# verdurin/pbdagcon

Hardware: AMD Instinct MI355X
Metric: consensus bases/sec (whole node) (higher is better)
Workload: dtype u8

## Files before the change

pbdagcon_amd/csrc/k_build.hip.h:

```cpp
#pragma once
#include <hip/hip_runtime.h>
#include "dagcon_dev.h"

#define DG_WAVE 64
#ifndef DG_LPW
#define DG_LPW 8u
#endif

__device__ __forceinline__ bool dg_failed(const DgParams &p) {
    return __hip_atomic_load(&p.st->err_flags, __ATOMIC_RELAXED, __HIP_MEMORY_SCOPE_AGENT) != 0;
}
__device__ __forceinline__ void dg_fail(const DgParams &p, uint32_t bit) {
    atomicOr(&p.st->err_flags, bit);
}
__device__ __forceinline__ void dg_fail_target(const DgParams &p, uint32_t t, uint32_t bit) {
    atomicOr(&p.tfail[t], bit);
}
__device__ __forceinline__ bool dg_tskip(const DgParams &p, uint32_t t) {
    return !p.tactive[t] || __hip_atomic_load(&p.tfail[t], __ATOMIC_RELAXED, __HIP_MEMORY_SCOPE_AGENT) != 0;
}
__device__ __forceinline__ bool dg_askip(const DgParams &p, uint32_t a) {
    return !(p.flags & DG_F_A1_ONLY) && __hip_atomic_load(&p.tfail[p.aln_tgt[a]], __ATOMIC_RELAXED, __HIP_MEMORY_SCOPE_AGENT) != 0;
}
__device__ __forceinline__ void dg_fail_aln(const DgParams &p, uint32_t a, uint32_t bit) {
    if (p.flags & DG_F_A1_ONLY) dg_fail(p, bit);
    else dg_fail_target(p, p.aln_tgt[a], bit);
    p.st->bad_aln = a;
}

#define DG_COL(qb, tb) ((uint16_t)((uint16_t)(qb) | ((uint16_t)(tb) << 8)))
#define DG_Q(c) ((uint8_t)((c) & 0xff))
#define DG_T(c) ((uint8_t)((c) >> 8))
#define DG_NW 64u
#define DG_NW_BIG 512u
#define DG_REDO 0xFFFFFFFFu

template <typename CT>
__device__ __forceinline__ void dg_store_run(const DgParams &p, CT *cell, const uint32_t run) {
    if constexpr (sizeof(CT) == 1) {
        if (run > 255u) { dg_fail(p, DG_E_RUN_WIDE); return; }
    }
    *cell = (CT)run;
}

template <typename CT>
__device__ inline void dg_finish_alignment(const DgParams &p, uint32_t a, uint16_t *buf, uint32_t m) {
    const uint32_t trim = p.trim;
    uint32_t lbases = 0, rbases = 0, lo = 0, hi = m;
    uint32_t start = p.aln_start[a];
    while (lbases < trim && lo < m) {
        if (DG_T(buf[lo++]) != DG_GAP) lbases++;
    }
    while (rbases < trim && hi > lo) {
        if (DG_T(buf[--hi]) != DG_GAP) rbases++;
    }
    start += lbases;
    const bool graph = !(p.flags & DG_F_A1_ONLY);
    uint32_t t_idx = 0, r = 0;
    CT *Cm = nullptr;
    if (graph) {
        t_idx = p.aln_tgt[a];
        if (p.tactive[t_idx]) {
            const uint64_t ab = p.aln_begin[t_idx];
            r = (uint32_t)(a - ab);
            Cm = static_cast<CT *>(p.matC) + p.matc_base[t_idx] + (uint64_t)r * p.matc_stride[t_idx];
        }
    }
    const uint32_t tlen = graph ? p.tlen[t_idx] : 0xFFFFFFFFu;
    uint32_t n_ins = 0, n_del = 0, adv = 0, run = 0;
    bool conf = start >= 1;
    uint32_t i = lo;
#define DG_FIN_COL(c, ci_)                                                                \
    do {                                                                                  \
        const uint8_t qb_ = DG_Q(c), tb_ = DG_T(c);                                       \
        if (qb_ == tb_ || qb_ == DG_GAP) {                                                \
            if (Cm && conf && ((start + adv) & ((1u << p.emit_shift) - 1u)) == 0 && start + adv <= tlen + 1) \
                ck[(start + adv) >> p.emit_shift] = ci_ - run;                            \
            if (run) { if (Cm && conf && start + adv <= tlen + 1) dg_store_run(p, Cm + (start + adv), run); run = 0; } \
            adv++; n_del += (qb_ != tb_);                                                 \
            if ((uint64_t)start - 1 + adv > (uint64_t)tlen) conf = false;                 \
        } else if (tb_ == DG_GAP) { n_ins++; run++; }                                     \
    } while (0)
    uint32_t *ck = p.ckpt + p.ck_base[a];
    while (i < hi && (i & 7u)) { const uint16_t c = buf[i]; DG_FIN_COL(c, i); i++; }
    while (i + 8 <= hi) {
        const uint4 v = *reinterpret_cast<const uint4 *>(buf + i);
        const uint32_t w4[4] = {v.x, v.y, v.z, v.w};
#pragma unroll
        for (int k = 0; k < 4; k++) {
            const uint16_t c0 = (uint16_t)(w4[k] & 0xffffu), c1 = (uint16_t)(w4[k] >> 16);
            DG_FIN_COL(c0, i + 2 * k);
            DG_FIN_COL(c1, i + 2 * k + 1);
        }
        i += 8;
    }
    while (i < hi) { const uint16_t c = buf[i]; DG_FIN_COL(c, i); i++; }
    if (run && Cm && conf && ((start + adv) & ((1u << p.emit_shift) - 1u)) == 0 && start + adv <= tlen + 1)
        ck[(start + adv) >> p.emit_shift] = hi - run;
    if (run && Cm && conf && start + adv <= tlen + 1) dg_store_run(p, Cm + (start + adv), run);
#undef DG_FIN_COL
    p.n_lo[a] = lo; p.n_hi[a] = hi; p.n_start[a] = start;
    p.n_ins[a] = n_ins; p.n_del[a] = n_del;
    atomicAdd(&p.st->n_columns, (unsigned long long)(hi - lo));
    if (graph && hi > lo && !conf) dg_fail_aln(p, a, DG_E_NONCONF);
}

#ifndef DG_NCH
#define DG_NCH 512u
#endif
#define DG_CH_NONE 0xFFFFFFFFu

__device__ __forceinline__ bool dg_match_col(uint8_t qb, uint8_t tb) { return qb == tb && qb != DG_GAP && qb != '.'; }

__device__ inline uint32_t dg_chunk_start(const uint8_t *q, const uint8_t *t, uint32_t len, uint32_t c) {
    if (c == 0) return 0;
    const uint64_t w0 = (uint64_t)c * DG_NCH;
    if (w0 >= len) return DG_CH_NONE;
    const uint32_t hi = (uint64_t)len < w0 + DG_NCH ? len : (uint32_t)(w0 + DG_NCH);
    for (uint32_t k = (uint32_t)w0; k < hi; k++) {
        const uint8_t b = q[k];
        if (dg_match_col(b, t[k]) && b != q[k - 1] && dg_match_col(q[k - 1], t[k - 1]) && dg_match_col(q[k - 2], t[k - 2]))
            return k;
    }
    return DG_CH_NONE;
}

struct DgChunkRun { uint32_t w, tb; bool dirty, overflow, badchar; };

template <uint32_t NW>
__device__ inline DgChunkRun dg_norm_run(const uint8_t *q, const uint8_t *t, const uint32_t len, const uint32_t k0,
                                         const uint32_t k1, uint16_t *win, uint16_t *out) {
#define DG_W(x) win[(x) & (NW - 1u)]
    DgChunkRun r;
    r.w = 0; r.tb = 0; r.dirty = false; r.overflow = false; r.badchar = false;
    if (k0 >= k1) return r;
    uint32_t badw = 0;
    uint32_t ip = k0, e = 0, i = 0, w = 0, tb = 0, jt = 0, jq = 0;
    uint32_t e_end = 0xFFFFFFFFu;
    uint32_t o0 = 0, o1 = 0, o2 = 0, o3 = 0;
    uint32_t in_done = 0, dirty = 0, overflow = 0;
    for (;;) {
        asm volatile("" : "+v"(in_done), "+v"(dirty));
        if (!in_done && (e - i) + 32u > NW) { overflow = 1; break; }
        if (!in_done) {
            uint32_t take = len - ip;
            if (take > 16u) take = 16u;
            if (ip < k1 && take > k1 - ip) take = k1 - ip;
#define DG_EXPAND(QB, TB)                                                      \
            do {                                                               \
                uint8_t qb_ = (QB), tb_ = (TB);                                \
                if (qb_ == '.') qb_ = DG_GAP;                                  \
                if (tb_ == '.') tb_ = DG_GAP;                                  \
                 \
                                   \
                const bool mm_ = qb_ != tb_ && qb_ != DG_GAP && tb_ != DG_GAP; \
                DG_W(e) = mm_ ? DG_COL(DG_GAP, tb_) : DG_COL(qb_, tb_);        \
                DG_W(e + 1u) = DG_COL(qb_, DG_GAP);                            \
                e += mm_ ? 2u : 1u;                                            \
            } while (0)
            if (take == 16u && (((uintptr_t)(q + ip)) & 15u) == 0) {
                const uint4 qv = *reinterpret_cast<const uint4 *>(q + ip);
                const uint4 tv = *reinterpret_cast<const uint4 *>(t + ip);
                const uint32_t qw[4] = {qv.x, qv.y, qv.z, qv.w}, tw[4] = {tv.x, tv.y, tv.z, tv.w};
#pragma unroll
                for (int k = 0; k < 4; k++) {
                    badw |= ((qw[k] - 0x21212121u) & ~qw[k]) | ((qw[k] + 0x01010101u) | qw[k]);
                    badw |= ((tw[k] - 0x21212121u) & ~tw[k]) | ((tw[k] + 0x01010101u) | tw[k]);
                }
#pragma unroll
                for (int k = 0; k < 16; k++)
                    DG_EXPAND((uint8_t)(qw[k >> 2] >> (8 * (k & 3))), (uint8_t)(tw[k >> 2] >> (8 * (k & 3))));
            } else {
                const uint32_t to_align = (uint32_t)((16u - (((uintptr_t)(q + ip)) & 15u)) & 15u);
                if (to_align && take > to_align) take = to_align;
                for (uint32_t k = 0; k < take; k++) {
                    const uint8_t qb0 = q[ip + k], tb0 = t[ip + k];
                    if (qb0 < 33 || qb0 > 126 || tb0 < 33 || tb0 > 126) badw = 0x80u;
                    DG_EXPAND(qb0, tb0);
                }
            }
#undef DG_EXPAND
            ip += take;
            if (ip == k1) e_end = e;
            if (ip == len) in_done = 1;
        }
        while (i < e && i < e_end) {
            if (i + 1 == e && !in_done) break;
            const uint16_t c = DG_W(i);
            uint8_t qi = DG_Q(c), ti = DG_T(c);
            uint32_t more = 0;
            if (i + 1 < e) {
                if (ti == DG_GAP) {
                    if (jt <= i) jt = i + 1;
                    while (jt < e && DG_T(DG_W(jt)) == DG_GAP) jt++;
                    if (jt < e) {
                        const uint16_t cj = DG_W(jt);
                        if (DG_T(cj) == qi) { ti = qi; DG_W(jt) = DG_COL(DG_Q(cj), DG_GAP); dirty |= (uint32_t)(jt >= e_end); }
                    } else if (!in_done) more = 2;
                }
                if (!more && qi == DG_GAP) {
                    if (jq <= i) jq = i + 1;
                    while (jq < e && DG_Q(DG_W(jq)) == DG_GAP) jq++;
                    if (jq < e) {
                        const uint16_t cj = DG_W(jq);
                        if (DG_Q(cj) == ti) { qi = ti; DG_W(jq) = DG_COL(DG_GAP, DG_T(cj)); dirty |= (uint32_t)(jq >= e_end); }
                    } else if (!in_done) more = 2;
                }
            }
            if (more) { DG_W(i) = DG_COL(qi, ti); break; }
            if (qi != DG_GAP || ti != DG_GAP) {
                o0 = (o0 >> 16) | (o1 << 16); o1 = (o1 >> 16) | (o2 << 16); o2 = (o2 >> 16) | (o3 << 16);
                o3 = (o3 >> 16) | ((uint32_t)DG_COL(qi, ti) << 16);
                w++;
                tb += (ti != DG_GAP);
                if ((w & 7u) == 0) *reinterpret_cast<uint4 *>(out + w - 8) = make_uint4(o0, o1, o2, o3);
            }
            i++;
        }
        if (i == e_end) break;
    }
#undef DG_W
    for (uint32_t k = w & 7u, x = w - (w & 7u); k > 0; k--, x++) {
        const uint32_t sh = 8u - k;
        const uint32_t word = sh >> 1;
        const uint32_t v = word == 0 ? o0 : word == 1 ? o1 : word == 2 ? o2 : o3;
        out[x] = (uint16_t)((sh & 1u) ? v >> 16 : v & 0xffffu);
    }
    r.w = w; r.tb = tb; r.dirty = dirty != 0; r.overflow = overflow != 0; r.badchar = (badw & 0x80808080u) != 0;
    return r;
}

template <uint32_t NW, uint32_t LANES, bool RETRY>
__global__ __launch_bounds__(LANES) void k_norm_chunk(DgParams p) {
    __shared__ uint16_t s_win[LANES * (NW + 2u)];
    const uint32_t g = threadIdx.x * gridDim.x + blockIdx.x;
    if (g >= p.n_chunks) return;
    if (dg_failed(p)) return;
    if (RETRY && p.ch_flag[g] != 2u) return;
    const uint32_t a = p.ch_aln[g];
    if (dg_askip(p, a)) { if (!RETRY) p.ch_flag[g] = 0; return; }
    const uint32_t c = g - p.ch_base[a], nwin = p.ch_base[a + 1] - p.ch_base[a];
    const uint64_t off = p.aln_off[a];
    const uint32_t len = p.aln_len[a];
    const uint8_t *q = p.q + off, *t = p.t + off;
    uint32_t flag = 0;
    DgChunkRun r;
    r.w = 0; r.tb = 0; r.dirty = false; r.overflow = false; r.badchar = false;
    uint32_t k0 = DG_CH_NONE, cn = c + 1;
    uint64_t src = 0;
    if (p.flags & DG_F_RAW) {
        if (c == 0) { k0 = 0; cn = nwin; flag = 1; }
    } else {
        k0 = dg_chunk_start(q, t, len, c);
        if (k0 != DG_CH_NONE) {
            uint16_t *win = s_win + threadIdx.x * (NW + 2u);
            src = (2ull * (off + k0) + 8ull * g + 7ull) & ~7ull;
            for (;;) {
                uint32_t k1 = len;
                for (; cn < nwin; cn++) {
                    const uint32_t s = dg_chunk_start(q, t, len, cn);
                    if (s != DG_CH_NONE) { k1 = s; break; }
                }
                r = dg_norm_run<NW>(q, t, len, k0, k1, win, p.norm_tmp + src);
                if (r.badchar) dg_fail_aln(p, a, DG_E_BADCHAR);
                if (r.overflow) { flag = RETRY ? 1u : 2u; break; }
                if (!r.dirty) break;
                cn++;
                uint32_t k2 = len;
                for (uint32_t x = cn; x < nwin; x++) {
                    const uint32_t s = dg_chunk_start(q, t, len, x);
                    if (s != DG_CH_NONE) { k2 = s; break; }
                }
                const unsigned long long need = (2ull * (k2 - k0) + 15ull) & ~7ull;
                const unsigned long long o = atomicAdd(&p.st->ovf_top, need);
                if (p.tmp_main + o + need > p.tmp_cap) { flag = 1; break; }
                src = p.tmp_main + o;
            }
        }
    }
    p.ch_k0[g] = k0; p.ch_next[g] = cn; p.ch_w[g] = r.w; p.ch_tb[g] = r.tb;
    p.ch_flag[g] = flag; p.ch_src[g] = src;
}

__global__ __launch_bounds__(64) void k_norm_scan(DgParams p) {
    const uint32_t a = blockIdx.x * 64 + threadIdx.x;
    if (a >= p.A) return;
    if (dg_failed(p)) return;
    if (dg_askip(p, a)) return;
    const uint32_t g0 = p.ch_base[a], g1 = p.ch_base[a + 1];
    bool redo = false;
    uint32_t m = 0, tbt = 0;
    for (uint32_t g = g0; g < g1;) {
        if (p.ch_k0[g] == DG_CH_NONE) { p.ch_out[g] = DG_CH_NONE; g++; continue; }
        redo |= p.ch_flag[g] != 0;
        p.ch_out[g] = m; p.ch_adv[g] = tbt;
        m += p.ch_w[g]; tbt += p.ch_tb[g];
        uint32_t nx = g0 + p.ch_next[g];
        if (nx > g1) nx = g1;
        for (uint32_t x = g + 1; x < nx; x++) p.ch_out[x] = DG_CH_NONE;
        g = nx;
    }
    if (redo) { p.n_hi[a] = DG_REDO; return; }
    const uint32_t trim = p.trim;
    uint32_t lbases = 0, rbases = 0, lo = 0, hi = m;
    for (uint32_t g = g0; g < g1 && lbases < trim && lo < m; g++) {
        if (p.ch_out[g] == DG_CH_NONE) continue;
        const uint32_t w = p.ch_w[g], tb = p.ch_tb[g];
        if (lbases + tb < trim) { lo += w; lbases += tb; continue; }
        const uint16_t *src = p.norm_tmp + p.ch_src[g];
        for (uint32_t x = 0; x < w && lbases < trim; x++) {
            if (DG_T(src[x]) != DG_GAP) lbases++;
            lo++;
        }
    }
    for (uint32_t g = g1; g > g0 && rbases < trim && hi > lo;) {
        g--;
        const uint32_t o = p.ch_out[g];
        if (o == DG_CH_NONE) continue;
        const uint32_t tb = p.ch_tb[g];
        if (o >= lo && rbases + tb < trim) { hi = o; rbases += tb; continue; }
        const uint16_t *src = p.norm_tmp + p.ch_src[g];
        while (rbases < trim && hi > lo && hi > o) {
            if (DG_T(src[--hi - o]) != DG_GAP) rbases++;
        }
    }
    p.n_lo[a] = lo; p.n_hi[a] = hi; p.n_start[a] = p.aln_start[a] + lbases; p.n_lb[a] = lbases;
    p.n_ins[a] = 0; p.n_del[a] = 0;
    atomicAdd(&p.st->n_columns, (unsigned long long)(hi - lo));
}

__device__ __forceinline__ uint4 dg_funnel_cols(const uint4 A, const uint4 B, const uint32_t h) {
    const bool w1 = (h >> 1) & 1u, w2 = (h >> 2) & 1u, half = h & 1u;
    const uint32_t u0 = w1 ? A.y : A.x, u1 = w1 ? A.z : A.y, u2 = w1 ? A.w : A.z, u3 = w1 ? B.x : A.w,
                   u4 = w1 ? B.y : B.x, u5 = w1 ? B.z : B.y, u6 = w1 ? B.w : B.z;
    const uint32_t t0 = w2 ? u2 : u0, t1 = w2 ? u3 : u1, t2 = w2 ? u4 : u2, t3 = w2 ? u5 : u3, t4 = w2 ? u6 : u4;
    uint4 r;
    r.x = half ? __builtin_amdgcn_alignbit(t1, t0, 16) : t0;
    r.y = half ? __builtin_amdgcn_alignbit(t2, t1, 16) : t1;
    r.z = half ? __builtin_amdgcn_alignbit(t3, t2, 16) : t2;
    r.w = half ? __builtin_amdgcn_alignbit(t4, t3, 16) : t3;
    return r;
}

__device__ __forceinline__ uint32_t dg_wave_excl(const uint32_t v, const int lane) {
    int incl = (int)v;
    incl += __builtin_amdgcn_update_dpp(0, incl, 0x111, 0xf, 0xf, false);
    incl += __builtin_amdgcn_update_dpp(0, incl, 0x112, 0xf, 0xf, false);
    incl += __builtin_amdgcn_update_dpp(0, incl, 0x114, 0xf, 0xf, false);
    incl += __builtin_amdgcn_update_dpp(0, incl, 0x118, 0xf, 0xf, false);
    incl += __builtin_amdgcn_update_dpp(0, incl, 0x142, 0xa, 0xf, false);
    incl += __builtin_amdgcn_update_dpp(0, incl, 0x143, 0xc, 0xf, false);
    (void)lane;
    return (uint32_t)incl - v;
}

template <typename CT>
__global__ __launch_bounds__(256) void k_norm_finish2(DgParams p) {
    const uint32_t g = blockIdx.x * 4u + (threadIdx.x >> 6);
    if (g >= p.n_chunks) return;
    if (dg_failed(p)) return;
    const int lane = threadIdx.x & 63;
    const uint32_t a = p.ch_aln[g];
    if (dg_askip(p, a)) return;
    const uint32_t o = p.ch_out[g];
    if (o == DG_CH_NONE) return;
    const uint32_t hi = p.n_hi[a];
    if (hi == DG_REDO) return;
    const uint32_t lo = p.n_lo[a], start = p.n_start[a], lb = p.n_lb[a];
    const uint32_t w = p.ch_w[g], adv0 = p.ch_adv[g];
    const uint16_t *src = p.norm_tmp + p.ch_src[g];
    const uint4 *src4 = reinterpret_cast<const uint4 *>(src);
    uint16_t *dst = p.norm + p.norm_off[a] + o;
    const bool graph = !(p.flags & DG_F_A1_ONLY);
    uint32_t t_idx = 0;
    CT *Cm = nullptr;
    if (graph) {
        t_idx = p.aln_tgt[a];
        if (p.tactive[t_idx]) Cm = static_cast<CT *>(p.matC) + p.matc_base[t_idx] + (uint64_t)(a - p.aln_begin[t_idx]) * p.matc_stride[t_idx];
    }
    const uint32_t tlen = graph ? p.tlen[t_idx] : 0xFFFFFFFFu;
    uint32_t *ck = p.ckpt + p.ck_base[a];
    const uint32_t ck_mask = (1u << p.emit_shift) - 1u;
    const uint32_t adv_init = adv0 > lb ? adv0 - lb : 0u;
    const uint32_t f0 = lo > o ? lo - o : 0u;
    const uint32_t f1 = hi > o ? (hi - o < w ? hi - o : w) : 0u;
    const bool any = f1 > f0;
    const uint32_t fspan = any ? f1 - f0 : 0u;
#define DG_FIN_CONF(A) (start >= 1u && ((A) == 0u || (uint64_t)start - 1u + (A) <= (uint64_t)tlen))
    const uint32_t h0 = (8u - (o & 7u)) & 7u;
    const uint32_t h = h0 < w ? h0 : w;
    const uint32_t nb = (w - h) / 8u, nvec = (w + 7u) / 8u;
    if ((uint32_t)lane < h) dst[lane] = src[lane];
    { const uint32_t x = h + 8u * nb + (uint32_t)lane; if (lane < 8 && x < w) dst[x] = src[x]; }
    uint4 *dst4 = reinterpret_cast<uint4 *>(dst + h);
    uint32_t adv_tile = adv_init, run_tile = 0, n_ins = 0, n_del = 0;
    for (uint32_t v0 = 0; v0 < nvec; v0 += 64u) {
        const uint32_t vl = v0 + (uint32_t)lane;
        const uint4 pc = vl < nvec ? src4[vl] : make_uint4(0, 0, 0, 0);
        const uint4 pn = vl + 1 < nvec ? src4[vl + 1] : make_uint4(0, 0, 0, 0);
        if (vl < nb) dst4[vl] = dg_funnel_cols(pc, pn, h);
        if (!any || 8u * v0 >= f1) continue;
        uint32_t advm = 0, insm = 0, delm = 0;
#pragma unroll
        for (uint32_t k = 0; k < 8u; k++) {
            const uint32_t wd = ((k >> 1) & 3u) == 0 ? pc.x : ((k >> 1) & 3u) == 1 ? pc.y : ((k >> 1) & 3u) == 2 ? pc.z : pc.w;
            const uint16_t c = (uint16_t)((k & 1u) ? wd >> 16 : wd & 0xffffu);
            const bool inw = 8u * vl + k < 8u * nvec && 8u * vl + k - f0 < fspan;
            const uint8_t qb = DG_Q(c), tb = DG_T(c);
            const bool adv = inw && (qb == tb || qb == DG_GAP);
            advm |= adv ? 1u << k : 0u;
            delm |= (adv && qb != tb) ? 1u << k : 0u;
            insm |= (inw && !adv && tb == DG_GAP) ? 1u << k : 0u;
        }
        const uint32_t nadv = (uint32_t)__popc(advm), nI = (uint32_t)__popc(insm);
        n_ins += nI; n_del += (uint32_t)__popc(delm);
        const uint32_t adv_lane = adv_tile + dg_wave_excl(nadv, lane);
        uint32_t sf = advm ? 1u : 0u;
        uint32_t sv = advm ? (uint32_t)__popc(insm & ~((2u << (31 - __clz((int)advm))) - 1u)) : nI;
#pragma unroll
        for (int d = 1; d < 64; d <<= 1) {
            const uint32_t pf = (uint32_t)__shfl_up((int)sf, d), pv = (uint32_t)__shfl_up((int)sv, d);
            if (lane >= d) { sv = sf ? sv : pv + sv; sf |= pf; }
        }
        uint32_t ef = (uint32_t)__shfl_up((int)sf, 1), ev = (uint32_t)__shfl_up((int)sv, 1);
        if (lane == 0) { ef = 0; ev = 0; }
        uint32_t run = ef ? ev : ev + run_tile;
        const uint32_t lf = (uint32_t)__builtin_amdgcn_readlane((int)sf, 63), lv = (uint32_t)__builtin_amdgcn_readlane((int)sv, 63);
        run_tile = lf ? lv : lv + run_tile;
        adv_tile += (uint32_t)__builtin_amdgcn_readlane((int)(adv_lane - adv_tile + nadv), 63);
        uint32_t adv = adv_lane;
        if (Cm && (advm | insm)) {
#pragma unroll
            for (uint32_t k = 0; k < 8u; k++) {
                if ((advm >> k) & 1u) {
                    const bool conf = DG_FIN_CONF(adv);
                    const uint32_t x = 8u * vl + k;
                    if (conf && ((start + adv) & ck_mask) == 0 && start + adv <= tlen + 1 && !(x == 0 && o > lo))
                        ck[(start + adv) >> p.emit_shift] = o + x - run;
                    if (run && conf && start + adv <= tlen + 1) dg_store_run(p, Cm + (start + adv), run);
                    run = 0;
                    adv++;
                } else if ((insm >> k) & 1u) run++;
            }
        }
    }
    {
        const uint32_t adv = adv_tile, run = run_tile;
        const bool conf = DG_FIN_CONF(adv);
        if (lane == 0) {
            if (any && Cm && conf && ((start + adv) & ck_mask) == 0 && start + adv <= tlen + 1 && (o + f1 < hi || run))
                ck[(start + adv) >> p.emit_shift] = o + f1 - run;
            if (run && Cm && conf && start + adv <= tlen + 1) dg_store_run(p, Cm + (start + adv), run);
            if (graph && any && !conf) dg_fail_aln(p, a, DG_E_NONCONF);
        }
    }
    {
        const uint32_t ti = dg_wave_excl(n_ins, lane) + n_ins, td = dg_wave_excl(n_del, lane) + n_del;
        if (lane == 63) { if (ti) atomicAdd(&p.n_ins[a], ti); if (td) atomicAdd(&p.n_del[a], td); }
    }
#undef DG_FIN_CONF
}

template <typename CT>
__global__ __launch_bounds__(64) void k_normalize_slow(DgParams p) {
    const uint32_t a = blockIdx.x * 64 + threadIdx.x;
    if (a >= p.A) return;
    if (dg_failed(p)) return;
    if (dg_askip(p, a)) return;
    if (p.n_hi[a] != DG_REDO) return;
    const uint64_t off = p.aln_off[a];
    const uint32_t len = p.aln_len[a];
    const uint8_t *q = p.q + off, *t = p.t + off;
    uint16_t *buf = p.norm + p.norm_off[a];
    const bool raw = (p.flags & DG_F_RAW) != 0;
    uint32_t n = 0;
    for (uint32_t i = 0; i < len; i++) {
        uint8_t qb = q[i], tb = t[i];
        if (qb < 33 || qb > 126 || tb < 33 || tb > 126) dg_fail_aln(p, a, DG_E_BADCHAR);
        if (!raw) {
            if (qb == '.') qb = DG_GAP;
            if (tb == '.') tb = DG_GAP;
            if (qb != tb && qb != DG_GAP && tb != DG_GAP) {
                buf[n++] = DG_COL(DG_GAP, tb);
                buf[n++] = DG_COL(qb, DG_GAP);
                continue;
            }
        }
        buf[n++] = DG_COL(qb, tb);
    }
    uint32_t m = n;
    if (!raw) {
        uint32_t w = 0, jt = 0, jq = 0;
        for (uint32_t i = 0; i < n; i++) {
            uint16_t c = buf[i];
            uint8_t qi = DG_Q(c), ti = DG_T(c);
            if (i + 1 < n) {
                if (ti == DG_GAP) {
                    if (jt <= i) jt = i + 1;
                    while (jt < n && DG_T(buf[jt]) == DG_GAP) jt++;
                    if (jt < n) {
                        uint16_t cj = buf[jt];
                        if (DG_T(cj) == qi) { ti = qi; buf[jt] = DG_COL(DG_Q(cj), DG_GAP); }
                    }
                }
                if (qi == DG_GAP) {
                    if (jq <= i) jq = i + 1;
                    while (jq < n && DG_Q(buf[jq]) == DG_GAP) jq++;
                    if (jq < n) {
                        uint16_t cj = buf[jq];
                        if (DG_Q(cj) == ti) { qi = ti; buf[jq] = DG_COL(DG_GAP, DG_T(cj)); }
                    }
                }
            }
            if (qi != DG_GAP || ti != DG_GAP) buf[w++] = DG_COL(qi, ti);
        }
        m = w;
    }
    dg_finish_alignment<CT>(p, a, buf, m);
}

__device__ __forceinline__ uint32_t dg_pool_words(uint32_t tlen, uint32_t n_ins, uint32_t n_del,
                                                  uint32_t k, uint32_t growth_pct, uint32_t *fixed_words) {
    const uint64_t capb = dg_capb(k);
    const uint64_t fixed = 3ull * n_ins + (uint64_t)(tlen + 2) * 3ull * capb;
    const uint64_t spill = 3ull * ((uint64_t)n_ins + n_del + 2ull * k) + 64ull;
    const uint64_t growth = (fixed * growth_pct) / 100ull + spill + 256ull;
    *fixed_words = (uint32_t)fixed;
    const uint64_t tot = fixed + growth;
    return tot > 0xFFFFFFF0ull ? 0xFFFFFFF0u : (uint32_t)tot;
}

__global__ __launch_bounds__(1024) void k_carve(DgParams p) {
    __shared__ unsigned long long s_scan[1024];
    __shared__ unsigned long long s_carry_nodes, s_carry_pool;
    if (dg_failed(p)) return;
    const uint32_t tid = threadIdx.x;
    if (tid == 0) { s_carry_nodes = 0; s_carry_pool = 0; }
    __syncthreads();
    for (uint32_t t0 = 0; t0 < p.T; t0 += 1024) {
        const uint32_t t = t0 + tid;
        unsigned long long nodes = 0, poolw = 0;
        uint32_t fixed_words = 0, ins = 0;
        if (t < p.T && !dg_tskip(p, t)) {
            uint32_t del = 0;
            const uint64_t b = p.aln_begin[t], e = p.aln_begin[t + 1];
            for (uint64_t a = b; a < e; a++) { ins += p.n_ins[a]; del += p.n_del[a]; }
            nodes = (unsigned long long)p.tlen[t] + 2ull + ins;
            poolw = dg_pool_words(p.tlen[t], ins, del, (uint32_t)(e - b), p.growth_pct, &fixed_words);
            if (nodes > DG_MAX_NODES || poolw > 0x3FFFFFFFull) {
                dg_fail_target(p, t, DG_E_TOO_BIG);
                nodes = 0; poolw = 0; fixed_words = 0;
            }
        }
        s_scan[tid] = nodes;
        __syncthreads();
        for (uint32_t o = 1; o < 1024; o <<= 1) {
            unsigned long long v = tid >= o ? s_scan[tid - o] : 0;
            __syncthreads();
            s_scan[tid] += v;
            __syncthreads();
        }
        unsigned long long node_excl = s_scan[tid] - nodes + s_carry_nodes;
        unsigned long long node_tot = s_scan[1023];
        __syncthreads();
        s_scan[tid] = poolw;
        __syncthreads();
// ... 752 lines not shown
```

Before: 350.3 million.

## Add bitmask gap-skipping normalization run for the 64-slot window path

Adds a new normalization routine for the default 64-entry window. It keeps per-column target-gap and query-gap bitmasks and uses ctz to jump straight to gap columns and their partners, instead of scanning every column with per-byte branches. Input expansion is rewritten with SWAR byte-compare masks, and output is emitted in 8-column blocks with a fast path for gap-free blocks. The kernel also gains a launch-bounds occupancy hint for the non-retry variant. The bit logic is intricate and could diverge from the original scan on edge cases. The tighter occupancy hint may force register spills.

```diff
diff --git a/pbdagcon_amd/csrc/k_build.hip.h b/pbdagcon_amd/csrc/k_build.hip.h
--- a/pbdagcon_amd/csrc/k_build.hip.h
+++ b/pbdagcon_amd/csrc/k_build.hip.h
@@ -1,6 +1,7 @@
 #pragma once
 #include <hip/hip_runtime.h>
 #include "dagcon_dev.h"
+#include "k_norm_run.hip.h"
 
 #define DG_WAVE 64
 #ifndef DG_LPW
@@ -28,9 +29,6 @@
     p.st->bad_aln = a;
 }
 
-#define DG_COL(qb, tb) ((uint16_t)((uint16_t)(qb) | ((uint16_t)(tb) << 8)))
-#define DG_Q(c) ((uint8_t)((c) & 0xff))
-#define DG_T(c) ((uint8_t)((c) >> 8))
 #define DG_NW 64u
 #define DG_NW_BIG 512u
 #define DG_REDO 0xFFFFFFFFu
@@ -105,133 +103,8 @@
     if (graph && hi > lo && !conf) dg_fail_aln(p, a, DG_E_NONCONF);
 }
 
-#ifndef DG_NCH
-#define DG_NCH 512u
-#endif
-#define DG_CH_NONE 0xFFFFFFFFu
-
-__device__ __forceinline__ bool dg_match_col(uint8_t qb, uint8_t tb) { return qb == tb && qb != DG_GAP && qb != '.'; }
-
-__device__ inline uint32_t dg_chunk_start(const uint8_t *q, const uint8_t *t, uint32_t len, uint32_t c) {
-    if (c == 0) return 0;
-    const uint64_t w0 = (uint64_t)c * DG_NCH;
-    if (w0 >= len) return DG_CH_NONE;
-    const uint32_t hi = (uint64_t)len < w0 + DG_NCH ? len : (uint32_t)(w0 + DG_NCH);
-    for (uint32_t k = (uint32_t)w0; k < hi; k++) {
-        const uint8_t b = q[k];
-        if (dg_match_col(b, t[k]) && b != q[k - 1] && dg_match_col(q[k - 1], t[k - 1]) && dg_match_col(q[k - 2], t[k - 2]))
-            return k;
-    }
-    return DG_CH_NONE;
-}
-
-struct DgChunkRun { uint32_t w, tb; bool dirty, overflow, badchar; };
-
-template <uint32_t NW>
-__device__ inline DgChunkRun dg_norm_run(const uint8_t *q, const uint8_t *t, const uint32_t len, const uint32_t k0,
-                                         const uint32_t k1, uint16_t *win, uint16_t *out) {
-#define DG_W(x) win[(x) & (NW - 1u)]
-    DgChunkRun r;
-    r.w = 0; r.tb = 0; r.dirty = false; r.overflow = false; r.badchar = false;
-    if (k0 >= k1) return r;
-    uint32_t badw = 0;
-    uint32_t ip = k0, e = 0, i = 0, w = 0, tb = 0, jt = 0, jq = 0;
-    uint32_t e_end = 0xFFFFFFFFu;
-    uint32_t o0 = 0, o1 = 0, o2 = 0, o3 = 0;
-    uint32_t in_done = 0, dirty = 0, overflow = 0;
-    for (;;) {
-        asm volatile("" : "+v"(in_done), "+v"(dirty));
-        if (!in_done && (e - i) + 32u > NW) { overflow = 1; break; }
-        if (!in_done) {
-            uint32_t take = len - ip;
-            if (take > 16u) take = 16u;
-            if (ip < k1 && take > k1 - ip) take = k1 - ip;
-#define DG_EXPAND(QB, TB)                                                      \
-            do {                                                               \
-                uint8_t qb_ = (QB), tb_ = (TB);                                \
-                if (qb_ == '.') qb_ = DG_GAP;                                  \
-                if (tb_ == '.') tb_ = DG_GAP;                                  \
-                 \
-                                   \
-                const bool mm_ = qb_ != tb_ && qb_ != DG_GAP && tb_ != DG_GAP; \
-                DG_W(e) = mm_ ? DG_COL(DG_GAP, tb_) : DG_COL(qb_, tb_);        \
-                DG_W(e + 1u) = DG_COL(qb_, DG_GAP);                            \
-                e += mm_ ? 2u : 1u;                                            \
-            } while (0)
-            if (take == 16u && (((uintptr_t)(q + ip)) & 15u) == 0) {
-                const uint4 qv = *reinterpret_cast<const uint4 *>(q + ip);
-                const uint4 tv = *reinterpret_cast<const uint4 *>(t + ip);
-                const uint32_t qw[4] = {qv.x, qv.y, qv.z, qv.w}, tw[4] = {tv.x, tv.y, tv.z, tv.w};
-#pragma unroll
-                for (int k = 0; k < 4; k++) {
-                    badw |= ((qw[k] - 0x21212121u) & ~qw[k]) | ((qw[k] + 0x01010101u) | qw[k]);
-                    badw |= ((tw[k] - 0x21212121u) & ~tw[k]) | ((tw[k] + 0x01010101u) | tw[k]);
-                }
-#pragma unroll
-                for (int k = 0; k < 16; k++)
-                    DG_EXPAND((uint8_t)(qw[k >> 2] >> (8 * (k & 3))), (uint8_t)(tw[k >> 2] >> (8 * (k & 3))));
-            } else {
-                const uint32_t to_align = (uint32_t)((16u - (((uintptr_t)(q + ip)) & 15u)) & 15u);
-                if (to_align && take > to_align) take = to_align;
-                for (uint32_t k = 0; k < take; k++) {
-                    const uint8_t qb0 = q[ip + k], tb0 = t[ip + k];
-                    if (qb0 < 33 || qb0 > 126 || tb0 < 33 || tb0 > 126) badw = 0x80u;
-                    DG_EXPAND(qb0, tb0);
-                }
-            }
-#undef DG_EXPAND
-            ip += take;
-            if (ip == k1) e_end = e;
-            if (ip == len) in_done = 1;
-        }
-        while (i < e && i < e_end) {
-            if (i + 1 == e && !in_done) break;
-            const uint16_t c = DG_W(i);
-            uint8_t qi = DG_Q(c), ti = DG_T(c);
-            uint32_t more = 0;
-            if (i + 1 < e) {
-                if (ti == DG_GAP) {
-                    if (jt <= i) jt = i + 1;
-                    while (jt < e && DG_T(DG_W(jt)) == DG_GAP) jt++;
-                    if (jt < e) {
-                        const uint16_t cj = DG_W(jt);
-                        if (DG_T(cj) == qi) { ti = qi; DG_W(jt) = DG_COL(DG_Q(cj), DG_GAP); dirty |= (uint32_t)(jt >= e_end); }
-                    } else if (!in_done) more = 2;
-                }
-                if (!more && qi == DG_GAP) {
-                    if (jq <= i) jq = i + 1;
-                    while (jq < e && DG_Q(DG_W(jq)) == DG_GAP) jq++;
-                    if (jq < e) {
-                        const uint16_t cj = DG_W(jq);
-                        if (DG_Q(cj) == ti) { qi = ti; DG_W(jq) = DG_COL(DG_GAP, DG_T(cj)); dirty |= (uint32_t)(jq >= e_end); }
-                    } else if (!in_done) more = 2;
-                }
-            }
-            if (more) { DG_W(i) = DG_COL(qi, ti); break; }
-            if (qi != DG_GAP || ti != DG_GAP) {
-                o0 = (o0 >> 16) | (o1 << 16); o1 = (o1 >> 16) | (o2 << 16); o2 = (o2 >> 16) | (o3 << 16);
-                o3 = (o3 >> 16) | ((uint32_t)DG_COL(qi, ti) << 16);
-                w++;
-                tb += (ti != DG_GAP);
-                if ((w & 7u) == 0) *reinterpret_cast<uint4 *>(out + w - 8) = make_uint4(o0, o1, o2, o3);
-            }
-            i++;
-        }
-        if (i == e_end) break;
-    }
-#undef DG_W
-    for (uint32_t k = w & 7u, x = w - (w & 7u); k > 0; k--, x++) {
-        const uint32_t sh = 8u - k;
-        const uint32_t word = sh >> 1;
-        const uint32_t v = word == 0 ? o0 : word == 1 ? o1 : word == 2 ? o2 : o3;
-        out[x] = (uint16_t)((sh & 1u) ? v >> 16 : v & 0xffffu);
-    }
-    r.w = w; r.tb = tb; r.dirty = dirty != 0; r.overflow = overflow != 0; r.badchar = (badw & 0x80808080u) != 0;
-    return r;
-}
-
 template <uint32_t NW, uint32_t LANES, bool RETRY>
-__global__ __launch_bounds__(LANES) void k_norm_chunk(DgParams p) {
+__global__ __launch_bounds__(LANES, RETRY ? 1 : 5) void k_norm_chunk(DgParams p) {
     __shared__ uint16_t s_win[LANES * (NW + 2u)];
     const uint32_t g = threadIdx.x * gridDim.x + blockIdx.x;
     if (g >= p.n_chunks) return;
@@ -261,7 +134,8 @@
                     const uint32_t s = dg_chunk_start(q, t, len, cn);
                     if (s != DG_CH_NONE) { k1 = s; break; }
                 }
-                r = dg_norm_run<NW>(q, t, len, k0, k1, win, p.norm_tmp + src);
+                if constexpr (NW == DG_NW) r = dg_norm_run_gc(q, t, len, k0, k1, win, p.norm_tmp + src);
+                else r = dg_norm_run<NW>(q, t, len, k0, k1, win, p.norm_tmp + src);
                 if (r.badchar) dg_fail_aln(p, a, DG_E_BADCHAR);
                 if (r.overflow) { flag = RETRY ? 1u : 2u; break; }
                 if (!r.dirty) break;
diff --git a/pbdagcon_amd/csrc/k_norm_run.hip.h b/pbdagcon_amd/csrc/k_norm_run.hip.h
--- /dev/null
+++ b/pbdagcon_amd/csrc/k_norm_run.hip.h
@@ -0,0 +1,309 @@
+#pragma once
+#include <stddef.h>
+#include <stdint.h>
+
+#if defined(__HIPCC__)
+#include <hip/hip_runtime.h>
+#define DG_HD __host__ __device__
+#define DG_HD_INLINE __host__ __device__ __forceinline__
+typedef uint4 dg_u4;
+#define DG_MAKE_U4(a, b, c, d) make_uint4((a), (b), (c), (d))
+#else
+#define DG_HD
+#define DG_HD_INLINE inline __attribute__((always_inline))
+struct __attribute__((may_alias, aligned(16))) dg_u4 { uint32_t x, y, z, w; };
+static inline dg_u4 DG_MAKE_U4(uint32_t a, uint32_t b, uint32_t c, uint32_t d) { dg_u4 v; v.x = a; v.y = b; v.z = c; v.w = d; return v; }
+#endif
+#ifndef DG_GAP
+#define DG_GAP '-'
+#endif
+
+#define DG_COL(qb, tb) ((uint16_t)((uint16_t)(qb) | ((uint16_t)(tb) << 8)))
+#define DG_Q(c) ((uint8_t)((c) & 0xff))
+#define DG_T(c) ((uint8_t)((c) >> 8))
+
+#ifndef DG_NCH
+#define DG_NCH 512u
+#endif
+#define DG_CH_NONE 0xFFFFFFFFu
+
+DG_HD_INLINE bool dg_match_col(uint8_t qb, uint8_t tb) { return qb == tb && qb != DG_GAP && qb != '.'; }
+
+DG_HD inline uint32_t dg_chunk_start(const uint8_t *q, const uint8_t *t, uint32_t len, uint32_t c) {
+    if (c == 0) return 0;
+    const uint64_t w0 = (uint64_t)c * DG_NCH;
+    if (w0 >= len) return DG_CH_NONE;
+    const uint32_t hi = (uint64_t)len < w0 + DG_NCH ? len : (uint32_t)(w0 + DG_NCH);
+    for (uint32_t k = (uint32_t)w0; k < hi; k++) {
+        const uint8_t b = q[k];
+        if (dg_match_col(b, t[k]) && b != q[k - 1] && dg_match_col(q[k - 1], t[k - 1]) && dg_match_col(q[k - 2], t[k - 2]))
+            return k;
+    }
+    return DG_CH_NONE;
+}
+
+struct DgChunkRun { uint32_t w, tb; bool dirty, overflow, badchar; };
+
+template <uint32_t NW>
+DG_HD inline DgChunkRun dg_norm_run(const uint8_t *q, const uint8_t *t, const uint32_t len, const uint32_t k0,
+                                    const uint32_t k1, uint16_t *win, uint16_t *out) {
+#define DG_W(x) win[(x) & (NW - 1u)]
+    DgChunkRun r;
+    r.w = 0; r.tb = 0; r.dirty = false; r.overflow = false; r.badchar = false;
+    if (k0 >= k1) return r;
+    uint32_t badw = 0;
+    uint32_t ip = k0, e = 0, i = 0, w = 0, tb = 0, jt = 0, jq = 0;
+    uint32_t e_end = 0xFFFFFFFFu;
+    uint32_t o0 = 0, o1 = 0, o2 = 0, o3 = 0;
+    uint32_t in_done = 0, dirty = 0, overflow = 0;
+    for (;;) {
+#if defined(__HIP_DEVICE_COMPILE__)
+        asm volatile("" : "+v"(in_done), "+v"(dirty));
+#endif
+        if (!in_done && (e - i) + 32u > NW) { overflow = 1; break; }
+        if (!in_done) {
+            uint32_t take = len - ip;
+            if (take > 16u) take = 16u;
+            if (ip < k1 && take > k1 - ip) take = k1 - ip;
+#define DG_EXPAND(QB, TB)                                                      \
+            do {                                                               \
+                uint8_t qb_ = (QB), tb_ = (TB);                                \
+                if (qb_ == '.') qb_ = DG_GAP;                                  \
+                if (tb_ == '.') tb_ = DG_GAP;                                  \
+                 \
+                                   \
+                const bool mm_ = qb_ != tb_ && qb_ != DG_GAP && tb_ != DG_GAP; \
+                DG_W(e) = mm_ ? DG_COL(DG_GAP, tb_) : DG_COL(qb_, tb_);        \
+                DG_W(e + 1u) = DG_COL(qb_, DG_GAP);                            \
+                e += mm_ ? 2u : 1u;                                            \
+            } while (0)
+            if (take == 16u && (((uintptr_t)(q + ip)) & 15u) == 0) {
+                const dg_u4 qv = *reinterpret_cast<const dg_u4 *>(q + ip);
+                const dg_u4 tv = *reinterpret_cast<const dg_u4 *>(t + ip);
+                const uint32_t qw[4] = {qv.x, qv.y, qv.z, qv.w}, tw[4] = {tv.x, tv.y, tv.z, tv.w};
+#pragma unroll
+                for (int k = 0; k < 4; k++) {
+                    badw |= ((qw[k] - 0x21212121u) & ~qw[k]) | ((qw[k] + 0x01010101u) | qw[k]);
+                    badw |= ((tw[k] - 0x21212121u) & ~tw[k]) | ((tw[k] + 0x01010101u) | tw[k]);
+                }
+#pragma unroll
+                for (int k = 0; k < 16; k++)
+                    DG_EXPAND((uint8_t)(qw[k >> 2] >> (8 * (k & 3))), (uint8_t)(tw[k >> 2] >> (8 * (k & 3))));
+            } else {
+                const uint32_t to_align = (uint32_t)((16u - (((uintptr_t)(q + ip)) & 15u)) & 15u);
+                if (to_align && take > to_align) take = to_align;
+                for (uint32_t k = 0; k < take; k++) {
+                    const uint8_t qb0 = q[ip + k], tb0 = t[ip + k];
+                    if (qb0 < 33 || qb0 > 126 || tb0 < 33 || tb0 > 126) badw = 0x80u;
+                    DG_EXPAND(qb0, tb0);
+                }
+            }
+#undef DG_EXPAND
+            ip += take;
+            if (ip == k1) e_end = e;
+            if (ip == len) in_done = 1;
+        }
+        while (i < e && i < e_end) {
+            if (i + 1 == e && !in_done) break;
+            const uint16_t c = DG_W(i);
+            uint8_t qi = DG_Q(c), ti = DG_T(c);
+            uint32_t more = 0;
+            if (i + 1 < e) {
+                if (ti == DG_GAP) {
+                    if (jt <= i) jt = i + 1;
+                    while (jt < e && DG_T(DG_W(jt)) == DG_GAP) jt++;
+                    if (jt < e) {
+                        const uint16_t cj = DG_W(jt);
+                        if (DG_T(cj) == qi) { ti = qi; DG_W(jt) = DG_COL(DG_Q(cj), DG_GAP); dirty |= (uint32_t)(jt >= e_end); }
+                    } else if (!in_done) more = 2;
+                }
+                if (!more && qi == DG_GAP) {
+                    if (jq <= i) jq = i + 1;
+                    while (jq < e && DG_Q(DG_W(jq)) == DG_GAP) jq++;
+                    if (jq < e) {
+                        const uint16_t cj = DG_W(jq);
+                        if (DG_Q(cj) == ti) { qi = ti; DG_W(jq) = DG_COL(DG_GAP, DG_T(cj)); dirty |= (uint32_t)(jq >= e_end); }
+                    } else if (!in_done) more = 2;
+                }
+            }
+            if (more) { DG_W(i) = DG_COL(qi, ti); break; }
+            if (qi != DG_GAP || ti != DG_GAP) {
+                o0 = (o0 >> 16) | (o1 << 16); o1 = (o1 >> 16) | (o2 << 16); o2 = (o2 >> 16) | (o3 << 16);
+                o3 = (o3 >> 16) | ((uint32_t)DG_COL(qi, ti) << 16);
+                w++;
+                tb += (ti != DG_GAP);
+                if ((w & 7u) == 0) *reinterpret_cast<dg_u4 *>(out + w - 8) = DG_MAKE_U4(o0, o1, o2, o3);
+            }
+            i++;
+        }
+        if (i == e_end) break;
+    }
+#undef DG_W
+    for (uint32_t k = w & 7u, x = w - (w & 7u); k > 0; k--, x++) {
+        const uint32_t sh = 8u - k;
+        const uint32_t word = sh >> 1;
+        const uint32_t v = word == 0 ? o0 : word == 1 ? o1 : word == 2 ? o2 : o3;
+        out[x] = (uint16_t)((sh & 1u) ? v >> 16 : v & 0xffffu);
+    }
+    r.w = w; r.tb = tb; r.dirty = dirty != 0; r.overflow = overflow != 0; r.badchar = (badw & 0x80808080u) != 0;
+    return r;
+}
+
+DG_HD_INLINE uint32_t dg_eq_bytes(const uint32_t x, const uint32_t y) {
+    const uint32_t d = x ^ y;
+    return ~(((d & 0x7F7F7F7Fu) + 0x7F7F7F7Fu) | d) & 0x80808080u;
+}
+
+DG_HD inline DgChunkRun dg_norm_run_gc(const uint8_t *q, const uint8_t *t, const uint32_t len, const uint32_t k0,
+                                       const uint32_t k1, uint16_t *win, uint16_t *out) {
+#define DG_W(x) win[(x) & 63u]
+    DgChunkRun r;
+    r.w = 0; r.tb = 0; r.dirty = false; r.overflow = false; r.badchar = false;
+    if (k0 >= k1) return r;
+    uint32_t badw = 0;
+    uint32_t ip = k0, e = 0, i = 0, o = 0, w = 0, tb = 0;
+    uint32_t e_end = 0xFFFFFFFFu;
+    uint64_t TG = 0, QG = 0;
+    uint32_t in_done = 0, dirty = 0, overflow = 0;
+    for (;;) {
+#if defined(__HIP_DEVICE_COMPILE__)
+        asm volatile("" : "+v"(in_done), "+v"(dirty));
+#endif
+        if (!in_done && (e - o) + 32u > 64u) { overflow = 1; break; }
+        if (!in_done) {
+            uint32_t take = len - ip;
+            if (take > 16u) take = 16u;
+            if (ip < k1 && take > k1 - ip) take = k1 - ip;
+            uint32_t tgl = 0, qgl = 0, l = 0;
+            const uint32_t e0 = e, re0 = e - o;
+#define DG_FLAGS(QW, TW)                                                       \
+            const uint32_t qd_ = (QW) - (dg_eq_bytes((QW), 0x2E2E2E2Eu) >> 7), td_ = (TW) - (dg_eq_bytes((TW), 0x2E2E2E2Eu) >> 7); \
+            const uint32_t gq_ = dg_eq_bytes(qd_, 0x2D2D2D2Du), gt_ = dg_eq_bytes(td_, 0x2D2D2D2Du);                                  \
+            const uint32_t mmw_ = ~(dg_eq_bytes(qd_, td_) | gq_ | gt_) & 0x80808080u;                                                 \
+            const uint32_t X_ = (gt_ >> 7) | (mmw_ >> 6), Y_ = (gq_ | mmw_) >> 7
+#define DG_EXPAND(SH)                                                          \
+            do {                                                               \
+                const uint32_t qb_ = (qd_ >> (SH)) & 0xffu, tb_ = (td_ >> (SH)) & 0xffu;          \
+                const uint32_t nm_ = (uint32_t)((int32_t)(mmw_ << (24u - (SH))) >> 31);    \
+                const uint32_t x_ = e0 + l;                                    \
+                DG_W(x_) = (uint16_t)(((qb_ & ~nm_) | ((uint32_t)DG_GAP & nm_)) | (tb_ << 8));    \
+                DG_W(x_ + 1u) = (uint16_t)(qb_ | ((uint32_t)DG_GAP << 8));     \
+                tgl |= ((X_ >> (SH)) & 3u) << l;                               \
+                qgl |= ((Y_ >> (SH)) & 1u) << l;                               \
+                l += 1u - nm_;                                                 \
+            } while (0)
+            if (take == 16u && (((uintptr_t)(q + ip)) & 15u) == 0) {
+                const dg_u4 qv = *reinterpret_cast<const dg_u4 *>(q + ip);
+                const dg_u4 tv = *reinterpret_cast<const dg_u4 *>(t + ip);
+                const uint32_t qw[4] = {qv.x, qv.y, qv.z, qv.w}, tw[4] = {tv.x, tv.y, tv.z, tv.w};
+#pragma unroll
+                for (int k = 0; k < 4; k++) {
+                    badw |= ((qw[k] - 0x21212121u) & ~qw[k]) | ((qw[k] + 0x01010101u) | qw[k]);
+                    badw |= ((tw[k] - 0x21212121u) & ~tw[k]) | ((tw[k] + 0x01010101u) | tw[k]);
+                    DG_FLAGS(qw[k], tw[k]);
+                    DG_EXPAND(0u); DG_EXPAND(8u); DG_EXPAND(16u); DG_EXPAND(24u);
+                }
+            } else {
+                const uint32_t to_align = (uint32_t)((16u - (((uintptr_t)(q + ip)) & 15u)) & 15u);
+                if (to_align && take > to_align) take = to_align;
+                for (uint32_t k = 0; k < take; k++) {
+                    const uint32_t qb0 = q[ip + k], tb0 = t[ip + k];
+                    if (qb0 < 33 || qb0 > 126 || tb0 < 33 || tb0 > 126) badw = 0x80u;
+                    DG_FLAGS(qb0, tb0);
+                    DG_EXPAND(0u);
+                }
+            }
+#undef DG_EXPAND
+#undef DG_FLAGS
+            e = e0 + l;
+            TG |= (uint64_t)tgl << re0;
+            QG |= (uint64_t)qgl << re0;
+            ip += take;
+            if (ip == k1) e_end = e;
+            if (ip == len) in_done = 1;
+        }
+        const uint32_t lim = e < e_end ? e : e_end;
+        while (i < lim) {
+            const uint64_t m = ((TG | QG) >> (i - o)) & (~0ull >> (64u - (lim - i)));
+            if (!m) { i = lim; break; }
+            const uint32_t g = i + (uint32_t)__builtin_ctzll(m);
+            i = g;
+            if (g + 1u == e) {
+                if (in_done) i = g + 1u;
+                break;
+            }
+            const uint32_t rg = g - o;
+            const uint16_t c = DG_W(g);
+            uint8_t qi = DG_Q(c), ti = DG_T(c);
+            const uint64_t ahead = ~0ull >> (64u - ((e - o) - rg - 1u));
+            uint32_t more = 0;
+            if (ti == DG_GAP) {
+                const uint64_t nt = (~TG >> (rg + 1u)) & ahead;
+                if (nt) {
+                    const uint32_t d = rg + 1u + (uint32_t)__builtin_ctzll(nt);
+                    const uint16_t cj = DG_W(o + d);
+                    if (DG_T(cj) == qi) {
+                        ti = qi;
+                        DG_W(o + d) = DG_COL(DG_Q(cj), DG_GAP);
+                        DG_W(g) = DG_COL(qi, ti);
+                        TG ^= (1ull << rg) | (1ull << d);
+                        dirty |= (uint32_t)(o + d >= e_end);
+                    }
+                } else if (!in_done) more = 1;
+            }
+            if (!more && qi == DG_GAP) {
+                const uint64_t nq = (~QG >> (rg + 1u)) & ahead;
+                if (nq) {
+                    const uint32_t d = rg + 1u + (uint32_t)__builtin_ctzll(nq);
+                    const uint16_t cj = DG_W(o + d);
+                    if (DG_Q(cj) == ti) {
+                        qi = ti;
+                        DG_W(o + d) = DG_COL(DG_GAP, DG_T(cj));
+                        DG_W(g) = DG_COL(qi, ti);
+                        QG ^= (1ull << rg) | (1ull << d);
+                        dirty |= (uint32_t)(o + d >= e_end);
+                    }
+                } else if (!in_done) more = 1;
+            }
+            if (more) break;
+            i = g + 1u;
+        }
+        while (i - o >= 8u) {
+            if ((((uint32_t)TG & (uint32_t)QG) & 0xffu) == 0) {
+                uint32_t v[4];
+#pragma unroll
+                for (uint32_t k = 0; k < 4; k++) v[k] = (uint32_t)DG_W(o + 2u * k) | ((uint32_t)DG_W(o + 2u * k + 1u) << 16);
+                *reinterpret_cast<dg_u4 *>(out + w) = DG_MAKE_U4(v[0], v[1], v[2], v[3]);
+                tb += (uint32_t)__builtin_popcount(~(uint32_t)TG & 0xffu);
+                w += 8u; o += 8u;
+                TG >>= 8; QG >>= 8;
+            } else {
+                uint64_t nd = ~(TG & QG) & (~0ull >> (64u - (i - o)));
+                if (__builtin_popcountll(nd) < 8) break;
+                uint32_t d = 0;
+                for (uint32_t k = 0; k < 8u; k++) {
+                    d = (uint32_t)__builtin_ctzll(nd);
+                    nd &= nd - 1u;
+                    const uint16_t c = DG_W(o + d);
+                    out[w + k] = c;
+                    tb += (DG_T(c) != DG_GAP);
+                }
+                w += 8u; o += d + 1u;
+                TG = d + 1u < 64u ? TG >> (d + 1u) : 0;
+                QG = d + 1u < 64u ? QG >> (d + 1u) : 0;
+            }
+        }
+        if (i == e_end) break;
+    }
+    if (!overflow) {
+        for (uint32_t x = o; x < i; x++) {
+            const uint16_t c = DG_W(x);
+            if (c == DG_COL(DG_GAP, DG_GAP)) continue;
+            out[w++] = c;
+            tb += (DG_T(c) != DG_GAP);
+        }
+    }
+#undef DG_W
+    r.w = w; r.tb = tb; r.dirty = dirty != 0; r.overflow = overflow != 0; r.badchar = (badw & 0x80808080u) != 0;
+    return r;
+}
```

After: 365.3 million, median of 6. 4.3% higher.
